# liuzhenboo/Stereo-Visual-Odometry

Hardware: AMD Instinct MI355X
Metric: stereo frames/sec on KITTI-00 1241x376; LK-kernel achieved HBM GB/s vs peak (higher is better)
Workload: dtype u8; 1 GPU; S0 synthetic KITTI-like stereo sequence 1241x376 (config #2 stand-in), FAST+LK track_mode LK_stereof2f_pnp, batched frame pairs (256 per step, 4 distinct chunks cycled), frames resident in HBM for `value`; `m1` (--full) = host-resident frames, H2D included; pairs_ok_last_step=256, parallelism=1 GPU

## Files before the change

### stereo-visual-odometry_amd/csrc/lk.hip

```cpp
#include <cstring>
#include "lk_common.h"

namespace svo {

struct ExactTile {
    static constexpr int kColDw = 29, kTileDw = 28 * kColDw;
    static constexpr int kQPairs = 23, kJPairs = 27, kJMargin = 3;
    static constexpr bool kAlignedI = true;
};
constexpr int kLdsDwPerWave = kSlots * ExactTile::kTileDw;

#ifdef SVO_LK_STAMP
__device__ unsigned long long g_lk_stamp[2 * 1024];
__device__ __forceinline__ uint32_t lk_now() { return (uint32_t)__builtin_amdgcn_readfirstlane((int)(uint32_t)__builtin_amdgcn_s_memtime()); }
#define LK_STAMP_DECL uint32_t lk_t_ = 0, lk_acc_ = 0, lk_n_ = 0
#define LK_AT(i) do { if ((i) == SVO_LK_STAMP) lk_t_ = lk_now(); else if ((i) == SVO_LK_STAMP + 1) { lk_acc_ += lk_now() - lk_t_; lk_n_++; } } while (0)
#define LK_CALL_BEGIN do { if (SVO_LK_STAMP == 8) lk_t_ = lk_now(); } while (0)
#define LK_CALL_END(lane) do { if (SVO_LK_STAMP == 8) { lk_acc_ += lk_now() - lk_t_; lk_n_++; } \
    if ((lane) == 0) { atomicAdd(&g_lk_stamp[2 * (blockIdx.x & 1023)], (unsigned long long)lk_acc_); atomicAdd(&g_lk_stamp[2 * (blockIdx.x & 1023) + 1], (unsigned long long)lk_n_); } } while (0)
#else
#define LK_STAMP_DECL
#define LK_AT(i)
#define LK_CALL_BEGIN
#define LK_CALL_END(lane)
#endif


struct PixLane { int row, seg; uint32_t onmask, qoff; };

template <bool EDGE>
__device__ __forceinline__ void patch_slot(uint32_t tile_addr, const PixLane &pl, uint32_t Wau,
                                           uint32_t Wbu, int ipx, int ipy, int w, int h,
                                           uint32_t (&IxP)[4], uint32_t (&IyP)[4], int &nIIx, int &nIIy,
                                           int &pA11, int &pA12, int &pA22)
{
    uint32_t IvP[4];
    const uint32_t Wa = Wau & pl.onmask, Wb = Wbu & pl.onmask;
    uint32_t Q12[10], DX[8], DY[8];
    scharr_columns<10, ExactTile::kColDw, EDGE>((lds_cu32 *)(size_t)(tile_addr + pl.qoff), ipx + pl.seg * 7, ipy + pl.row, w, h, Q12, DX, DY);
    int iv[8], ix[8], iy[8];
    iv[7] = ix[7] = iy[7] = 0;
    patch_samples<10>(Q12, DX, DY, Wa, Wb, iv, ix, iy);
    pA11 = 0; pA12 = 0; pA22 = 0;
    int sIIx = 0, sIIy = 0;
#pragma unroll
    for (int m = 0; m < 4; m++) {
        IvP[m] = perm_b32((uint32_t)iv[2 * m + 1], (uint32_t)iv[2 * m], 0x05040100u);
        IxP[m] = perm_b32((uint32_t)ix[2 * m + 1], (uint32_t)ix[2 * m], 0x07060302u);
        IyP[m] = perm_b32((uint32_t)iy[2 * m + 1], (uint32_t)iy[2 * m], 0x07060302u);
        pA11 = m == 0 ? dot2_0(IxP[m], IxP[m]) : dot2(IxP[m], IxP[m], pA11);
        pA12 = m == 0 ? dot2_0(IxP[m], IyP[m]) : dot2(IxP[m], IyP[m], pA12);
        pA22 = m == 0 ? dot2_0(IyP[m], IyP[m]) : dot2(IyP[m], IyP[m], pA22);
        sIIx = m == 0 ? dot2_0(IvP[m], IxP[m]) : dot2(IvP[m], IxP[m], sIIx);
        sIIy = m == 0 ? dot2_0(IvP[m], IyP[m]) : dot2(IvP[m], IyP[m], sIIy);
    }
    nIIx = -sIIx; nIIy = -sIIy;
}

__device__ __forceinline__ void mismatch_slot(const uint32_t (&C)[8], uint32_t Wa, uint32_t Wb,
                                              const uint32_t (&IxP)[4], const uint32_t (&IyP)[4], int nIIx, int nIIy,
                                              int vround, int &pb1, int &pb2)
{
    int d[7];
#pragma unroll
    for (int k = 0; k < 7; k++) d[k] = dot2(C[k + 1], Wb, dot2_sv(C[k], Wa, vround));
#pragma unroll
    for (int m = 0; m < 4; m++) {
        const uint32_t vp = m < 3 ? perm_b32((uint32_t)d[2 * m + 1], (uint32_t)d[2 * m], 0x07060302u)
                                  : (uint32_t)d[6] >> 16;
        pb1 = m == 0 ? dot2_v(vp, IxP[m], nIIx) : dot2(vp, IxP[m], pb1);
        pb2 = m == 0 ? dot2_v(vp, IyP[m], nIIy) : dot2(vp, IyP[m], pb2);
    }
}


__device__ __forceinline__ void lk_call4(const PyrGeom &g, const uint8_t *slotI, const uint8_t *slotJ, float2 prevPt,
                                         float2 &outPt, int &status, bool live, uint32_t *lds, const uint32_t *lds_wg,
                                         int wave_off, int lane)
{
    typedef ExactTile T;
    LK_STAMP_DECL;
    LK_CALL_BEGIN;
    PixLane pl;
    pl.row = min(lane / 3, kWin - 1); pl.seg = lane - (lane / 3) * 3; pl.onmask = lane < 63 ? ~0u : 0u;
    pl.qoff = (uint32_t)((pl.seg * 7 * T::kColDw + pl.row) * 4);
    asm volatile("" : "+v"(pl.onmask));

    uint32_t IxP[kSlots][4], IyP[kSlots][4];
    int nIIx[kSlots], nIIy[kSlots];
    const int lane_off = (pl.seg * 7 * T::kColDw + pl.row) * 4 + wave_off;
    const StageLane q = stage_lane<T::kColDw>(lane);
    const uint32_t lds_base = (uint32_t)(size_t)(lds_cu32 *)lds;
    const int vround = j_sample_rounding();
    status = 1;
    float nx = 0.f, ny = 0.f;
    uint32_t rI[kSlots][3][2];
    request_I<T>(rI, g, g.nlevels - 1, slotI, prevPt, live, q, lane);
    for (int level = g.nlevels - 1; level >= 0; --level) {
        LK_AT(0);
        LkLevel lv = level_begin<T>(g, level, prevPt, live, nx, ny, status);
        bool lvl_on = lv.on;
        const int w = lv.w, h = lv.h, pitch = g.pitch[level];
        const int offI = (lv.ipx - 1) - i_tile_x0<T>(lv.ipx);
        const unsigned long long m_on = __ballot(lvl_on), m_j = __ballot(lv.tx0 != kNoJTile);
        uint32_t q_src[3];
        stage_src(q_src, q, pitch);
        uint32_t rJ[kSlots][3][2];
        int pA[kSlots][3];
#pragma unroll
        for (int s = 0; s < kSlots; s++) {
            if (!((m_on >> (16 * s)) & 1ull)) continue;
            tile_store_i<T>(lds + s * T::kTileDw, rI[s], q, lane);
        }
#pragma unroll
        for (int s = 0; s < kSlots; s++) {
            if (!((m_j >> (16 * s)) & 1ull)) continue;
            tile_request<T::kJPairs>(rJ[s], g, level, pitch, slotJ, lv.tx0, lv.ty0, s, q_src, lane);
        }
        wave_lds_fence();
        LK_AT(1);
#pragma unroll
        for (int s = 0; s < kSlots; s++) {
            pA[s][0] = pA[s][1] = pA[s][2] = 0;
            if (!((m_on >> (16 * s)) & 1ull)) continue;
            const uint32_t qaddr = lds_base + (uint32_t)((s * T::kTileDw + __builtin_amdgcn_readlane(offI, 16 * s) * T::kColDw) * 4);
            const uint32_t W01s = __builtin_amdgcn_readlane(lv.WIa, 16 * s), W23s = __builtin_amdgcn_readlane(lv.WIb, 16 * s);
            const int ipxs = __builtin_amdgcn_readlane(lv.ipx, 16 * s), ipys = __builtin_amdgcn_readlane(lv.ipy, 16 * s);
            if (__builtin_expect(ipxs < 0 || ipxs + kWin >= w || ipys < 0 || ipys + kWin >= h, 0))
                patch_slot<true>(qaddr, pl, W01s, W23s, ipxs, ipys, w, h, IxP[s], IyP[s], nIIx[s], nIIy[s],
                                 pA[s][0], pA[s][1], pA[s][2]);
            else
                patch_slot<false>(qaddr, pl, W01s, W23s, ipxs, ipys, w, h, IxP[s], IyP[s], nIIx[s], nIIy[s],
                                  pA[s][0], pA[s][1], pA[s][2]);
        }
        LK_AT(2);
        wave_lds_fence();
#pragma unroll
        for (int s = 0; s < kSlots; s++) {
            if (!((m_j >> (16 * s)) & 1ull)) continue;
            tile_store_j<T, false>(lds + s * T::kTileDw, rJ[s], q, lane);
        }
        wave_lds_fence();
        float A11, A12, A22;
        {
            int v1[8], v2[8];
#pragma unroll
            for (int s = 0; s < kSlots; s++) {
                v1[2 * s] = pA[s][0]; v1[2 * s + 1] = pA[s][1];
                v2[2 * s] = pA[s][2]; v2[2 * s + 1] = 0;
            }
            const int r1 = reduce_scatter8_rows(v1, lane), r2 = reduce_scatter8_rows(v2, lane);
            A11 = wide_to_f32(quad_bcast<2>(r1), quad_bcast<0>(r1)) * kFltScale;
            A12 = wide_to_f32(quad_bcast<3>(r1), quad_bcast<1>(r1)) * kFltScale;
            A22 = wide_to_f32(quad_bcast<2>(r2), quad_bcast<0>(r2)) * kFltScale;
        }
        float Dinv;
        lvl_on = level_solve_setup(A11, A12, A22, level, lvl_on, status, Dinv);

        if (level > 0) request_I<T>(rI, g, level - 1, slotI, prevPt, live, q, lane);
        LK_AT(3);
        float pdx = 0.f, pdy = 0.f;
        bool it_on = lvl_on;
        for (int j = 0; j < kLkMaxIter; j++) {
            if (!__any(it_on)) break;
            LK_AT(4);
            const LkIter it = iter_begin<T>(lv.qx, lv.qy, w, h, level, lane, it_on, status, lv.tx0, lv.ty0);
            it_on = it.on;
            const unsigned long long m_it = __ballot(it_on), m_rs = __ballot(it.restage);
            if (__builtin_expect(m_rs != 0, 0)) {
#pragma unroll
                for (int s = 0; s < kSlots; s++) {
                    if (!((m_rs >> (16 * s)) & 1ull)) continue;
                    uint32_t r[3][2];
                    tile_request<T::kJPairs>(r, g, level, pitch, slotJ, lv.tx0, lv.ty0, s, q_src, lane);
                    tile_store_j<T, false>(lds + s * T::kTileDw, r, q, lane);
                }
                wave_lds_fence();
            }
            LK_AT(5);
            int pb[kSlots][2];
#pragma unroll
            for (int s = 0; s < kSlots; s++) {
                pb[s][0] = pb[s][1] = 0;
                if (!((m_it >> (16 * s)) & 1ull)) continue;
                const int joffs = __builtin_amdgcn_readlane(it.joff, 16 * s);
                const uint32_t Was = __builtin_amdgcn_readlane(it.Wa, 16 * s), Wbs = __builtin_amdgcn_readlane(it.Wb, 16 * s);
                lds_cu32 *pj = (lds_cu32 *)(size_t)((uint32_t)(size_t)(lds_cu32 *)lds_wg + (uint32_t)(joffs + lane_off));
                uint32_t C[8];
#pragma unroll
                for (int k = 0; k < 8; k++) C[k] = pj[k * T::kColDw];
                mismatch_slot(C, Was, Wbs, IxP[s], IyP[s], nIIx[s], nIIy[s], vround, pb[s][0], pb[s][1]);
            }
            LK_AT(6);
            float b1f, b2f;
            {
                int v[8];
#pragma unroll
                for (int s = 0; s < kSlots; s++) { v[2 * s] = pb[s][0]; v[2 * s + 1] = pb[s][1]; }
                const int r = reduce_scatter8_rows(v, lane);
                b1f = wide_to_f32(quad_bcast<2>(r), quad_bcast<0>(r)) * kFltScale;
                b2f = wide_to_f32(quad_bcast<3>(r), quad_bcast<1>(r)) * kFltScale;
            }
            it_on = iter_update(A11, A12, A22, Dinv, b1f, b2f, j, it_on, lv.qx, lv.qy, nx, ny, pdx, pdy);
            LK_AT(7);
        }
        final_window_check(nx, ny, w, h, level, live, status);
    }
    outPt = make_float2(nx, ny);
    LK_CALL_END(lane);
}

#ifndef SVO_LK_WAVES_PER_WG
#define SVO_LK_WAVES_PER_WG 1
#endif
constexpr int kLkWavesPerWg = SVO_LK_WAVES_PER_WG;
static_assert(kLkWavesPerWg == 4 || kLkWavesPerWg == 2 || kLkWavesPerWg == 1, "lk_kernel: 4, 2 or 1 waves per workgroup");
constexpr int kLkSpreadWavesPerWg = 4;

template <int W>
__global__ __launch_bounds__(64 * W) __attribute__((amdgpu_waves_per_eu(3, 3))) void lk_kernel(LkArgs a)
{
    __shared__ uint32_t lds[W * kLdsDwPerWave];
    const int wave = W == 1 ? 0 : (int)(threadIdx.x >> 6), lane = threadIdx.x & 63;
    uint32_t *my = lds + wave * kLdsDwPerWave;
    lk_track_item<W>(a, wave, lane, [&](const uint8_t *sI, const uint8_t *sJ, float2 cur, float2 &nxt, int &st, bool live) {
        lk_call4(a.g, sI, sJ, cur, nxt, st, live, my, lds, wave * (kLdsDwPerWave * 4), lane);
    });
}

__global__ __launch_bounds__(1024) void compact_kernel(CompactArgs a)
{
    __shared__ int wave_tot[16];
    __shared__ int base_s;
    const int b = blockIdx.x;
    int n = a.n_pts ? a.n_pts[b] : a.n_fixed;
    n = min(n, a.cap);
    const int lane = threadIdx.x & 63, wv = threadIdx.x >> 6;
    const int64_t o = (int64_t)b * a.pts_stride;
    if (threadIdx.x == 0) base_s = 0;
    __syncthreads();
    for (int start = 0; start < n; start += 1024) {
        int i = start + threadIdx.x;
        bool k = i < n && a.keep[o + i] != 0;
        unsigned long long m = __ballot(k);
        int rank = __popcll(m & ((1ull << lane) - 1ull));
        if (lane == 0) wave_tot[wv] = __popcll(m);
        __syncthreads();
        int pre = 0, tot = 0;
        for (int q = 0; q < 16; q++) { int t = wave_tot[q]; if (q < wv) pre += t; tot += t; }
        int dst = base_s + pre + rank;
        if (k) {
#pragma unroll
            for (int c = 0; c < 4; c++) a.out[c][o + dst] = a.in[c][o + i];
        }
        __syncthreads();
        if (threadIdx.x == 0) base_s += tot;
        __syncthreads();
    }
    if (threadIdx.x == 0) a.m_out[b] = base_s;
}

#ifdef SVO_LK_STAMP
extern "C" int svo_debug_lk_stamps(unsigned long long out[2], int reset)
{
    static unsigned long long h[2 * 1024];
    if (hipMemcpyFromSymbol(h, HIP_SYMBOL(g_lk_stamp), sizeof(h)) != hipSuccess) return -1;
    out[0] = out[1] = 0;
    for (int i = 0; i < 1024; i++) { out[0] += h[2 * i]; out[1] += h[2 * i + 1]; }
    if (reset) { memset(h, 0, sizeof(h)); if (hipMemcpyToSymbol(HIP_SYMBOL(g_lk_stamp), h, sizeof(h)) != hipSuccess) return -1; }
    return 0;
}
#endif

void launch_lk(const LkArgs &a0, int batch, int max_pts, hipStream_t st)
{
    if (max_pts <= 0 || batch <= 0) return;
    if (a0.accum != 0) { launch_lk_sse2(a0, batch, max_pts, st); return; }
    constexpr int W = kLkWavesPerWg;
// ... 24 lines not shown
```

### stereo-visual-odometry_amd/csrc/lk_common.h

```cpp
#pragma once
#include "svo_device.h"
#include "svo_kernels.h"

namespace svo {

constexpr int kSlots = 4;
constexpr int W_BITS = 14;
constexpr float kHalfWin = 10.f;
constexpr float kFltScale = 1.f / (1 << 20);
constexpr int kNoJTile = -(1 << 20);


typedef short s16x2 __attribute__((ext_vector_type(2)));
typedef unsigned short u16x2 __attribute__((ext_vector_type(2)));
typedef uint32_t u32_unaligned __attribute__((aligned(1)));
typedef const uint32_t __attribute__((address_space(3))) lds_cu32;

__device__ __forceinline__ int cv_floor(float v)
{
    int r;
    asm("v_cvt_flr_i32_f32 %0, %1" : "=v"(r) : "v"(v));
    return r;
}
__device__ __forceinline__ uint32_t perm_b32(uint32_t s0, uint32_t s1, uint32_t sel) { return __builtin_amdgcn_perm(s0, s1, sel); }
__device__ __forceinline__ int dot2(uint32_t a, uint32_t b, int c)
{
    return __builtin_amdgcn_sdot2(__builtin_bit_cast(s16x2, a), __builtin_bit_cast(s16x2, b), c, false);
}
__device__ __forceinline__ int dot2_k(uint32_t a, uint32_t b, int k)
{
    int r;
    asm("v_dot2_i32_i16 %0, %1, %2, %3" : "=v"(r) : "v"(a), "v"(b), "s"(k));
    return r;
}
__device__ __forceinline__ int dot2_0(uint32_t a, uint32_t b)
{
    int r;
    asm("v_dot2_i32_i16 %0, %1, %2, 0" : "=v"(r) : "v"(a), "v"(b));
    return r;
}
__device__ __forceinline__ uint32_t as_u32(u16x2 v) { return __builtin_bit_cast(uint32_t, v); }
__device__ __forceinline__ u16x2 as_u16x2(uint32_t v) { return __builtin_bit_cast(u16x2, v); }

__device__ __forceinline__ float wide_to_f32(int hi, int lo)
{
    return __builtin_fmaf((float)hi, 65536.f, (float)lo);
}
struct PackedWeights { uint32_t Wa, Wb; };
__device__ __forceinline__ PackedWeights bilinear_weights(float a, float b)
{
    const float magic = 12582912.f;
    const float a1 = 1.f - a, b1 = (1.f - b) * (float)(1 << W_BITS), b0 = b * (float)(1 << W_BITS);
    const uint32_t u00 = __float_as_uint(a1 * b1 + magic), u01 = __float_as_uint(a * b1 + magic),
                   u10 = __float_as_uint(a1 * b0 + magic);
    const uint32_t w11 = (uint32_t)(1 << W_BITS) + 3u * 0x4B400000u - u00 - u01 - u10;
    PackedWeights w;
    w.Wa = perm_b32(u10, u00, 0x05040100u);
    w.Wb = perm_b32(w11, u01, 0x05040100u);
    return w;
}

__device__ __forceinline__ bool window_oob(int ix, int iy, int w, int h)
{
    return (unsigned)(ix + kWin) >= (unsigned)(w + kWin) || (unsigned)(iy + kWin) >= (unsigned)(h + kWin);
}

__device__ __forceinline__ int dot2_v(uint32_t a, uint32_t b, int c)
{
    int r;
    asm("v_dot2_i32_i16 %0, %1, %2, %3" : "=v"(r) : "v"(a), "v"(b), "v"(c));
    return r;
}
__device__ __forceinline__ int dot2_sv(uint32_t a, uint32_t b_uniform, int c)
{
    int r;
    asm("v_dot2_i32_i16 %0, %1, %2, %3" : "=v"(r) : "v"(a), "s"(b_uniform), "v"(c));
    return r;
}
__device__ __forceinline__ int j_sample_rounding()
{
    int vround = 1 << (W_BITS - 5 - 1 + 7);
    asm volatile("" : "+v"(vround));
    return vround;
}

struct StageLane { int pr[3], dc4[3], dst[3]; };
template <int CS>
__device__ __forceinline__ StageLane stage_lane(int lane)
{
    StageLane q;
#pragma unroll
    for (int t = 0; t < 3; t++) {
        const int i = lane + 64 * t;
        q.pr[t] = i / 7; q.dc4[t] = 4 * (i - q.pr[t] * 7); q.dst[t] = q.dc4[t] * CS + q.pr[t];
    }
    return q;
}
__device__ __forceinline__ void stage_src(uint32_t (&src)[3], const StageLane &q, int pitch)
{
#pragma unroll
    for (int t = 0; t < 3; t++) src[t] = (uint32_t)(q.pr[t] * pitch + q.dc4[t]);
}
__device__ __forceinline__ void tile_loads(uint32_t (&r)[3][2], const uint8_t *rowA, const uint8_t *rowB, uint32_t s_off,
                                           const uint32_t (&q_src)[3], int lane, int n_items)
{
#pragma unroll
    for (int t = 0; t < 3; t++) {
        if (lane + 64 * t < n_items) {
            const uint32_t o = s_off + q_src[t];
            r[t][0] = *(const u32_unaligned *)(rowA + o); r[t][1] = *(const u32_unaligned *)(rowB + o);
        }
    }
}
template <int PAIRS>
__device__ __forceinline__ void tile_request(uint32_t (&r)[3][2], const PyrGeom &g, int level, int pitch, const uint8_t *slot,
                                             int x, int y, int s, const uint32_t (&q_src)[3], int lane)
{
// ... 28 lines not shown
                d[c * T::kColDw] = as_u32(as_u16x2(perm_b32(bot, top, 0x040c000cu + 0x01000100u * c)) >> one);
            }
        }
    }
}

template <int NC, int CS, bool EDGE>
__device__ __forceinline__ void scharr_columns(lds_cu32 *q0, int gx0, int gyA, int w, int h, uint32_t (&Q12)[NC],
                                               uint32_t (&DX)[NC - 2], uint32_t (&DY)[NC - 2])
{
    uint32_t Q01[NC], Q23[NC];
#pragma unroll
    for (int j = 0; j < NC; j++) { Q01[j] = q0[j * CS]; Q12[j] = q0[j * CS + 1]; Q23[j] = q0[j * CS + 2]; }
    uint32_t T0[NC], T1[NC];
    const u16x2 k12 = {12, 12}, k40 = {40, 40};
#pragma unroll
    for (int j = 0; j < NC; j++) {
        T0[j] = as_u32((as_u16x2(Q01[j]) + as_u16x2(Q23[j])) * k12 + as_u16x2(Q12[j]) * k40);
        T1[j] = as_u32(as_u16x2(Q23[j]) - as_u16x2(Q01[j]));
    }
#pragma unroll
    for (int c = 0; c < NC - 2; c++) {
        DX[c] = as_u32(as_u16x2(T0[c + 2]) - as_u16x2(T0[c]));
        DY[c] = as_u32((as_u16x2(T1[c]) + as_u16x2(T1[c + 2])) * k12 + as_u16x2(T1[c + 1]) * k40);
    }
    if (EDGE) {
        const int gyB = gyA + 1;
        const uint32_t rows = ((gyA >= 0 && gyA < h) ? 0x0000FFFFu : 0u) | ((gyB >= 0 && gyB < h) ? 0xFFFF0000u : 0u);
#pragma unroll
        for (int c = 0; c < NC - 2; c++) {
            const int gx = gx0 + c;
            const uint32_t mk = (gx >= 0 && gx < w) ? rows : 0u;
            DX[c] &= mk; DY[c] &= mk;
        }
    }
}
template <int NC>
__device__ __forceinline__ void patch_samples(const uint32_t (&Q12)[NC], const uint32_t (&DX)[NC - 2], const uint32_t (&DY)[NC - 2],
                                              uint32_t Wa, uint32_t Wb, int (&iv)[8], int (&ix)[8], int (&iy)[8])
{
#pragma unroll
    for (int k = 0; k < NC - 3; k++) {
        iv[k] = dot2(Q12[k + 2], Wb, dot2_k(Q12[k + 1], Wa, 1 << (W_BITS - 5 - 1))) >> (W_BITS - 5);
        ix[k] = dot2(DX[k + 1], Wb, dot2_k(DX[k], Wa, 1 << (W_BITS + 1)));
        iy[k] = dot2(DY[k + 1], Wb, dot2_k(DY[k], Wa, 1 << (W_BITS + 1)));
    }
}


template <class T> __device__ __forceinline__ int i_tile_x0(int ipx) { return T::kAlignedI ? (ipx - 1) & ~3 : ipx - 1; }

template <class T>
__device__ __forceinline__ void request_I(uint32_t (&rI)[kSlots][3][2], const PyrGeom &g, int level, const uint8_t *slotI,
                                          float2 prevPt, bool live, const StageLane &q, int lane)
{
    const float lscale = 1.f / (float)(1 << level);
    const int ipx = cv_floor(prevPt.x * lscale - kHalfWin), ipy = cv_floor(prevPt.y * lscale - kHalfWin);
    const int pitch = g.pitch[level];
    const unsigned long long m = __ballot(live && !window_oob(ipx, ipy, g.w[level], g.h[level]));
    const int x0 = i_tile_x0<T>(ipx), y0 = ipy - 1;
    uint32_t src[3];
    stage_src(src, q, pitch);
#pragma unroll
    for (int s = 0; s < kSlots; s++) {
        if (!((m >> (16 * s)) & 1ull)) continue;
        tile_request<T::kQPairs>(rI[s], g, level, pitch, slotI, x0, y0, s, src, lane);
    }
}

struct LkLevel {
    int w, h;
    int ipx, ipy;
    uint32_t WIa, WIb;
    bool on;
    float qx, qy;
    int tx0, ty0;
};
template <class T>
__device__ __forceinline__ LkLevel level_begin(const PyrGeom &g, int level, float2 prevPt, bool live, float &nx, float &ny,
                                               int &status)
{
    LkLevel v;
    v.w = g.w[level]; v.h = g.h[level];
    const float lscale = 1.f / (float)(1 << level);
    float px = prevPt.x * lscale, py = prevPt.y * lscale;
    if (level == g.nlevels - 1) { nx = px; ny = py; }
    else { nx = nx * 2.f; ny = ny * 2.f; }
    px -= kHalfWin; py -= kHalfWin;
    v.ipx = cv_floor(px); v.ipy = cv_floor(py);
    const bool oob = window_oob(v.ipx, v.ipy, v.w, v.h);
    if (live && oob && level == 0) status = 0;
    v.on = live && !oob;
    const PackedWeights wt = bilinear_weights(px - (float)v.ipx, py - (float)v.ipy);
    v.WIa = wt.Wa; v.WIb = wt.Wb;
    v.qx = nx - kHalfWin; v.qy = ny - kHalfWin;
    v.tx0 = kNoJTile; v.ty0 = 0;
    const int inx = cv_floor(v.qx), iny = cv_floor(v.qy);
    if (v.on && !window_oob(inx, iny, v.w, v.h)) { v.tx0 = inx - T::kJMargin; v.ty0 = iny - T::kJMargin; }
    return v;
}

__device__ __forceinline__ bool level_solve_setup(float A11, float A12, float A22, int level, bool lvl_on, int &status, float &Dinv)
{
    const float D = A11 * A22 - A12 * A12;
    const float minEig = (A22 + A11 - sqrtf((A11 - A22) * (A11 - A22) + 4.f * A12 * A12)) /
                         (float)(2 * kWin * kWin);
    const bool degenerate = minEig < 0.001f || D < 1.1920929e-07f;
    if (lvl_on && degenerate && level == 0) status = 0;
    Dinv = 1.f / D;
    return lvl_on && !degenerate;
}

struct LkIter {
    bool on;
    uint32_t Wa, Wb;
    int joff;
    bool restage;
};
template <class T>
__device__ __forceinline__ LkIter iter_begin(float qx, float qy, int w, int h, int level, int lane, bool it_on, int &status,
                                             int &tx0, int &ty0)
{
    LkIter it;
    const int inx = cv_floor(qx), iny = cv_floor(qy);
    if (it_on && window_oob(inx, iny, w, h)) {
        if (level == 0) status = 0;
        it_on = false;
    }
    const PackedWeights wj = bilinear_weights(qx - (float)inx, qy - (float)iny);
    it.Wa = wj.Wa; it.Wb = wj.Wb;
    int cx = inx - tx0, cy = iny - ty0;
    it.restage = it_on && ((unsigned)cx > (unsigned)(2 * T::kJMargin) || (unsigned)cy > (unsigned)(2 * T::kJMargin));
    if (it.restage) { tx0 = inx - T::kJMargin; ty0 = iny - T::kJMargin; cx = T::kJMargin; cy = T::kJMargin; }
    it.joff = ((int)__umul24((unsigned)cx, T::kColDw) + cy + (lane >> 4) * T::kTileDw) * 4;
    it.on = it_on;
    return it;
}

__device__ __forceinline__ bool iter_update(float A11, float A12, float A22, float Dinv, float b1f, float b2f, int j, bool it_on,
                                            float &qx, float &qy, float &nx, float &ny, float &pdx, float &pdy)
{
    const float dlx = (A12 * b2f - A22 * b1f) * Dinv;
    const float dly = (A12 * b1f - A11 * b2f) * Dinv;
    const float dd = dlx * dlx + dly * dly;
    bool conv = dd <= 0.9999e-4f;
    if (__builtin_expect(__any(it_on && !conv && dd < 1.0001e-4f), 0)) {
        asm volatile("" ::: "memory");
        conv = (double)dlx * (double)dlx + (double)dly * (double)dly <= 0.01 * 0.01;
    }
    if (it_on) {
        qx += dlx; qy += dly;
        nx = qx + kHalfWin; ny = qy + kHalfWin;
        if (conv) it_on = false;
        else if (j > 0 && fabsf(dlx + pdx) <= 0.01f && fabsf(dly + pdy) <= 0.01f) {
            nx -= dlx * 0.5f; ny -= dly * 0.5f;
            it_on = false;
        }
        pdx = dlx; pdy = dly;
    }
    return it_on;
}

__device__ __forceinline__ void final_window_check(float nx, float ny, int w, int h, int level, bool live, int &status)
{
    if (live && status && level == 0) {
        const int fx = cv_floor(nx - kHalfWin), fy = cv_floor(ny - kHalfWin);
        if (window_oob(fx, fy, w, h)) status = 0;
    }
}

struct LkItem { int b, bx; };
__device__ __forceinline__ LkItem lk_item_of_workgroup(const LkArgs &a)
{
    const int n_aware = (a.batch & ~7) * a.gx;
    LkItem it;
    if ((int)blockIdx.x < n_aware) {
        const int xcd = blockIdx.x & 7, slot_id = blockIdx.x >> 3;
        it.b = (slot_id / a.gx) * 8 + xcd; it.bx = slot_id % a.gx;
    } else {
        const int r = blockIdx.x - n_aware;
        it.b = (a.batch & ~7) + r / a.gx; it.bx = r % a.gx;
    }
    return it;
}

template <int W, class Call>
__device__ __forceinline__ void lk_track_item(const LkArgs &a, int wave, int lane, Call &&lk_call)
{
    const LkItem item = lk_item_of_workgroup(a);
    const int b = item.b, slot = lane >> 4;
    int n = a.n_pts ? a.n_pts[b] : a.n_fixed;
    n = min(n, a.cap);
    int spw = kSlots;
    if (a.spread) spw = min(kSlots, max(1, (n + a.gx * W - 1) / (a.gx * W)));
    for (int first = (item.bx * W + wave) * spw; first < n; first += a.gx * W * spw) {
        const int idx = first + slot;
        const bool valid = slot < spw && idx < n;
        const bool writer = valid && lane == 16 * slot;
        const int64_t po = (int64_t)b * a.pts_stride + (valid ? idx : first);
        const float2 p0 = a.pts_in[po];
        float2 cur = p0, nxt;
        bool outside = p0.x < 0 || p0.y < 0, bad = false, noepi = false;
        bool live = valid;
        float prev_y = p0.y;
#pragma nounroll
        for (int c = 0; c < a.ncalls; c++) {
            const uint8_t *sI = a.prev[c] + (int64_t)b * a.slot_stride;
            const uint8_t *sJ = a.next[c] + (int64_t)b * a.slot_stride;
            int st;
            lk_call(sI, sJ, cur, nxt, st, live);
            if (writer && live) {
                a.pts_out[c][po] = nxt;
                a.status[c][po] = (uint8_t)st;
            }
            if (live) {
                outside = outside || nxt.x < 0 || nxt.y < 0;
                bad = bad || st == 0;
                if (c == 0 || c == 2) noepi = noepi || (double)fabsf(prev_y - nxt.y) > a.match_err;
                prev_y = nxt.y;
                cur = nxt;
            }
            if (a.ncalls == 4 && (outside || bad || noepi)) live = false;
            if (!__any(live)) break;
        }
        if (a.ncalls == 4 && writer) a.keep[po] = !(outside || bad || noepi);
        wave_lds_fence();
    }
}

}
```

### stereo-visual-odometry_amd/csrc/lk_sse2.hip

```cpp
#include "lk_common.h"

namespace svo {

constexpr int kCS2 = 26, kJMargin2 = 2;
constexpr int kQPairs2 = 23, kJPairs2 = kWin + 2 * kJMargin2;
constexpr int kTileDw2 = 26 * kCS2, kTileSpill = 2 * kCS2;
constexpr int kTilesDw = kSlots * kTileDw2;
struct ChainTile {
    static constexpr int kColDw = kCS2, kTileDw = kTileDw2;
    static constexpr int kQPairs = kQPairs2, kJPairs = kJPairs2, kJMargin = kJMargin2;
    static constexpr bool kAlignedI = false;
};
constexpr int kStageDw = 576;
constexpr int kTailY = 0, kTailX = 416;
__device__ constexpr int kChainOff[8] = {108, 196, 372, 284, 328, 240, 524, 152};
constexpr int kAq0 = kTileSpill;
__host__ __device__ constexpr int a_stride(bool simd128) { return simd128 ? 84 : 108; }
__host__ __device__ constexpr int a_tail_base(bool simd128) { return kAq0 + 4 * a_stride(simd128); }
constexpr int kLdsDwSse2 = kTilesDw + kSlots * kStageDw + 16;
constexpr int kDumpB = kChainOff[0] + 43, kDumpA = kStageDw - 1;
constexpr int kStageDwL = 960, kTailYL = 180, kTailXL = 468;
__device__ constexpr int kChainOffL[8] = {88, 584, 0, 764, 676, 288, 376, 860};
constexpr int kLdsDwLegacy = kTilesDw + kSlots * kStageDwL + 16;
constexpr int kDumpBL = kChainOffL[0] + 87, kDumpAL = kStageDwL - 1;
// ... 196 lines not shown
#pragma unroll
    for (int i = 0; i < 3; i++)
#pragma unroll
        for (int e = 0; e < 4; e++)
            if (4 * i + e >= first && 4 * i + e < last) {
                const f32x2 f = {(float)(short)(q[i][e] & 0xFFFFu), (float)((int)q[i][e] >> 16)};
                d = pk_fma(f, f, d);
                m = __builtin_fmaf(f.x, f.y, m);
            }
}
__device__ __forceinline__ void chain_a(const Sse2Lane &L, float &s11, float &s12, float &s22)
{
    lds_cu32x4 *p = (lds_cu32x4 *)(size_t)L.ca;
    f32x2 d = {0.f, 0.f}, d21, d84 = {0.f, 0.f};
    float m = 0.f, m21, m84 = 0.f;
    u32x4 q[3], n[3];
#pragma unroll
    for (int i = 0; i < 3; i++) q[i] = p[i];
#pragma unroll
    for (int i = 0; i < 3; i++) n[i] = p[3 + i];
    asm volatile("" ::: "memory");
    a_terms(d, m, q, 0, 12);
#pragma unroll
    for (int i = 0; i < 3; i++) q[i] = p[6 + i];
    asm volatile("" ::: "memory");
    a_terms(d, m, n, 0, 9);
    d21 = d; m21 = m;
    a_terms(d, m, n, 9, 12);
#pragma nounroll
    for (int turn = 0; turn < 3; turn++, p += 6) {
#pragma unroll
        for (int i = 0; i < 3; i++) n[i] = p[9 + i];
        asm volatile("" ::: "memory");
        a_terms(d, m, q, 0, 12);
        if (turn == 2) { d84 = d; m84 = m; }
#pragma unroll
        for (int i = 0; i < 3; i++) q[i] = p[12 + i];
        asm volatile("" ::: "memory");
        a_terms(d, m, n, 0, 12);
    }
    a_terms(d, m, q, 0, 9);
    s11 = L.a_sel == 0 ? d21.x : (L.a_sel == 1 ? d84.x : d.x);
    s12 = L.a_sel == 0 ? m21 : (L.a_sel == 1 ? m84 : m);
    s22 = L.a_sel == 0 ? d21.y : (L.a_sel == 1 ? d84.y : d.y);
}
__device__ __forceinline__ float combine_a(float r)
{
    const float u = ((r + row_shl<1>(r)) + row_shl<2>(r)) + row_shl<3>(r);
    return row_first(row_shl<4>(r) + u);
}

template <bool LEGACY>
__device__ __forceinline__ void lk_call4_sse2(const PyrGeom &g, const uint8_t *slotI, const uint8_t *slotJ, float2 prevPt,
                                              float2 &outPt, int &status, bool live, uint32_t *lds, int lane,
                                              const Sse2Lane &L)
{
    typedef ChainTile T;
    uint32_t IvP[kSlots][4], IxP[kSlots][4], IyP[kSlots][4], Ix4[kSlots], Iy4[kSlots];
    const StageLane q = stage_lane<T::kColDw>(lane);
    const uint32_t lds_base = (uint32_t)(size_t)(lds_cu32 *)lds;
    const int vround = j_sample_rounding();
    status = 1;
    float nx = 0.f, ny = 0.f;
    uint32_t rI[kSlots][3][2];
    request_I<T>(rI, g, g.nlevels - 1, slotI, prevPt, live, q, lane);
    for (int level = g.nlevels - 1; level >= 0; --level) {
        LkLevel lv = level_begin<T>(g, level, prevPt, live, nx, ny, status);
        bool lvl_on = lv.on;
        const int w = lv.w, h = lv.h, pitch = g.pitch[level];
        const unsigned long long m_on = __ballot(lvl_on), m_j = __ballot(lv.tx0 != kNoJTile);
        uint32_t q_src[3];
        stage_src(q_src, q, pitch);
        uint32_t rJ[kSlots][3][2];
#pragma unroll
        for (int s = 0; s < kSlots; s++) {
            if (!((m_on >> (16 * s)) & 1ull)) continue;
            tile_store_i<T>(lds + s * T::kTileDw, rI[s], q, lane);
        }
#pragma unroll
        for (int s = 0; s < kSlots; s++) {
            if (!((m_j >> (16 * s)) & 1ull)) continue;
            tile_request<T::kJPairs>(rJ[s], g, level, pitch, slotJ, lv.tx0, lv.ty0, s, q_src, lane);
        }
        wave_lds_fence();
#pragma unroll
        for (int s = 0; s < kSlots; s++) {
            if (!((m_on >> (16 * s)) & 1ull)) continue;
            const uint32_t qaddr = lds_base + (uint32_t)(s * T::kTileDw * 4);
            const uint32_t W01s = __builtin_amdgcn_readlane(lv.WIa, 16 * s), W23s = __builtin_amdgcn_readlane(lv.WIb, 16 * s);
            const int ipxs = __builtin_amdgcn_readlane(lv.ipx, 16 * s), ipys = __builtin_amdgcn_readlane(lv.ipy, 16 * s);
            uint32_t Aw[8];
            if (__builtin_expect(ipxs < 0 || ipxs + kWin >= w || ipys < 0 || ipys + kWin >= h, 0))
                patch_slot8<true>(qaddr, L, W01s, W23s, ipxs, ipys, w, h, IvP[s], IxP[s], IyP[s], Ix4[s], Iy4[s], Aw);
            else
                patch_slot8<false>(qaddr, L, W01s, W23s, ipxs, ipys, w, h, IvP[s], IxP[s], IyP[s], Ix4[s], Iy4[s], Aw);
            const uint32_t so = (uint32_t)(s * stage_dw<LEGACY>() * 4);
#pragma unroll
            for (int i = 0; i < 8; i++) lds_store(L.wa[i] + so, Aw[i]);
        }
        wave_lds_fence();
#pragma unroll
        for (int s = 0; s < kSlots; s++) {
            if (!((m_j >> (16 * s)) & 1ull)) continue;
            tile_store_j<T, false>(lds + s * T::kTileDw, rJ[s], q, lane);
        }
        float A11, A12, A22;
        {
            float r11, r12, r22;
            chain_a(L, r11, r12, r22);
            A11 = combine_a(r11) * kFltScale;
            A12 = combine_a(r12) * kFltScale;
            A22 = combine_a(r22) * kFltScale;
        }
        wave_lds_fence();
        float Dinv;
        lvl_on = level_solve_setup(A11, A12, A22, level, lvl_on, status, Dinv);

        if (level > 0) request_I<T>(rI, g, level - 1, slotI, prevPt, live, q, lane);
        float pdx = 0.f, pdy = 0.f;
        bool it_on = lvl_on;
        for (int j = 0; j < kLkMaxIter; j++) {
            if (!__any(it_on)) break;
            const LkIter it = iter_begin<T>(lv.qx, lv.qy, w, h, level, lane, it_on, status, lv.tx0, lv.ty0);
            it_on = it.on;
            const unsigned long long m_it = __ballot(it_on), m_rs = __ballot(it.restage);
            if (__builtin_expect(m_rs != 0, 0)) {
#pragma unroll
                for (int s = 0; s < kSlots; s++) {
                    if (!((m_rs >> (16 * s)) & 1ull)) continue;
                    uint32_t r[3][2];
                    tile_request<T::kJPairs>(r, g, level, pitch, slotJ, lv.tx0, lv.ty0, s, q_src, lane);
                    tile_store_j<T, true>(lds + s * T::kTileDw, r, q, lane);
                }
                wave_lds_fence();
            }
#pragma unroll
            for (int s = 0; s < kSlots; s++) {
                if (!((m_it >> (16 * s)) & 1ull)) continue;
                const int joffs = __builtin_amdgcn_readlane(it.joff, 16 * s);
                const uint32_t Was = __builtin_amdgcn_readlane(it.Wa, 16 * s), Wbs = __builtin_amdgcn_readlane(it.Wb, 16 * s);
                lds_cu32 *pj = (lds_cu32 *)(size_t)(lds_base + (uint32_t)joffs + L.qoff);
                uint32_t C[9];
#pragma unroll
                for (int k = 0; k < 9; k++) C[k] = pj[k * T::kColDw];
                float v[16];
                mismatch_slot8<LEGACY>(C, Was, Wbs, IvP[s], IxP[s], IyP[s], Ix4[s], Iy4[s], vround, v);
                const uint32_t so = (uint32_t)(s * stage_dw<LEGACY>() * 4);
#pragma unroll
                for (int t = 0; t < (LEGACY ? 16 : 10); t++) lds_store(L.wb[t] + so, __float_as_uint(v[t]));
            }
            wave_lds_fence();
            float b1f, b2f;
            {
                const float r = chain_b<LEGACY>(L);
                const float bb = r + row_shl<1>(r);
                const float u = bb + row_shl<2>(bb);
                const float f = r + row_shl<1>(u);
                b1f = row_first(f) * kFltScale;
                b2f = row_first(row_shl<8>(f)) * kFltScale;
            }
            wave_lds_fence();
            it_on = iter_update(A11, A12, A22, Dinv, b1f, b2f, j, it_on, lv.qx, lv.qy, nx, ny, pdx, pdy);
        }
        final_window_check(nx, ny, w, h, level, live, status);
    }
    outPt = make_float2(nx, ny);
}

template <bool LEGACY>
__global__ __launch_bounds__(64) __attribute__((amdgpu_waves_per_eu(2, 2))) void lk_sse2_kernel(LkArgs a)
{
    __shared__ __attribute__((aligned(16))) uint32_t lds[LEGACY ? kLdsDwLegacy : kLdsDwSse2];
    const int lane = threadIdx.x & 63;
    const Sse2Lane L = make_lane<LEGACY>(lane, (uint32_t)(size_t)(lds_cu32 *)lds, a.accum == 2);
    lk_track_item<1>(a, 0, lane, [&](const uint8_t *sI, const uint8_t *sJ, float2 cur, float2 &nxt, int &st, bool live) {
        lk_call4_sse2<LEGACY>(a.g, sI, sJ, cur, nxt, st, live, lds, lane, L);
    });
}

void launch_lk_sse2(const LkArgs &a0, int batch, int max_pts, hipStream_t st)
{
    if (max_pts <= 0 || batch <= 0) return;
    const int waves = (max_pts + kSlots - 1) / kSlots;
    LkArgs a = a0;
    a.gx = waves < 768 ? waves : 768;
    a.spread = 0;
    if (batch < 4) {
        const int room = 2048 / batch;
        a.gx = max_pts < room ? max_pts : room;
        a.spread = 1;
    }
    a.batch = batch;
    if (a.accum == 3) {
        if (batch < 4) {
            const int room = 1536 / batch;
            a.gx = max_pts < room ? max_pts : room;
        }
        hipLaunchKernelGGL(lk_sse2_kernel<true>, dim3(batch * a.gx), dim3(64), 0, st, a);
    } else {
        hipLaunchKernelGGL(lk_sse2_kernel<false>, dim3(batch * a.gx), dim3(64), 0, st, a);
    }
}

}
```

Before: 18650 stereo pairs/s.

## Represent LK per-lane predicates as wave-wide lane masks instead of bools

```diff
diff --git a/stereo-visual-odometry_amd/csrc/lk.hip b/stereo-visual-odometry_amd/csrc/lk.hip
--- a/stereo-visual-odometry_amd/csrc/lk.hip
+++ b/stereo-visual-odometry_amd/csrc/lk.hip
@@ -74,8 +74,11 @@
 }
 
 
+__device__ __forceinline__ void undefined_sums(int &x, int &y) { asm("" : "=v"(x), "=v"(y)); }
+__device__ __forceinline__ void undefined_sums(int &x, int &y, int &z) { asm("" : "=v"(x), "=v"(y), "=v"(z)); }
+
 __device__ __forceinline__ void lk_call4(const PyrGeom &g, const uint8_t *slotI, const uint8_t *slotJ, float2 prevPt,
-                                         float2 &outPt, int &status, bool live, uint32_t *lds, const uint32_t *lds_wg,
+                                         float2 &outPt, lanemask &status, lanemask live, uint32_t *lds, const uint32_t *lds_wg,
                                          int wave_off, int lane)
 {
     typedef ExactTile T;
@@ -92,37 +95,37 @@
     const StageLane q = stage_lane<T::kColDw>(lane);
     const uint32_t lds_base = (uint32_t)(size_t)(lds_cu32 *)lds;
     const int vround = j_sample_rounding();
-    status = 1;
+    status = ~0ull;
     float nx = 0.f, ny = 0.f;
     uint32_t rI[kSlots][3][2];
     request_I<T>(rI, g, g.nlevels - 1, slotI, prevPt, live, q, lane);
     for (int level = g.nlevels - 1; level >= 0; --level) {
         LK_AT(0);
         LkLevel lv = level_begin<T>(g, level, prevPt, live, nx, ny, status);
-        bool lvl_on = lv.on;
+        lanemask lvl_on = lv.on;
         const int w = lv.w, h = lv.h, pitch = g.pitch[level];
         const int offI = (lv.ipx - 1) - i_tile_x0<T>(lv.ipx);
-        const unsigned long long m_on = __ballot(lvl_on), m_j = __ballot(lv.tx0 != kNoJTile);
+        const lanemask m_on = lvl_on, m_j = lv.j_staged;
         uint32_t q_src[3];
         stage_src(q_src, q, pitch);
         uint32_t rJ[kSlots][3][2];
         int pA[kSlots][3];
 #pragma unroll
         for (int s = 0; s < kSlots; s++) {
-            if (!((m_on >> (16 * s)) & 1ull)) continue;
+            if (!slot_bit(m_on, s)) continue;
             tile_store_i<T>(lds + s * T::kTileDw, rI[s], q, lane);
         }
 #pragma unroll
         for (int s = 0; s < kSlots; s++) {
-            if (!((m_j >> (16 * s)) & 1ull)) continue;
+            if (!slot_bit(m_j, s)) continue;
             tile_request<T::kJPairs>(rJ[s], g, level, pitch, slotJ, lv.tx0, lv.ty0, s, q_src, lane);
         }
         wave_lds_fence();
         LK_AT(1);
 #pragma unroll
         for (int s = 0; s < kSlots; s++) {
-            pA[s][0] = pA[s][1] = pA[s][2] = 0;
-            if (!((m_on >> (16 * s)) & 1ull)) continue;
+            undefined_sums(pA[s][0], pA[s][1], pA[s][2]);
+            if (!slot_bit(m_on, s)) continue;
             const uint32_t qaddr = lds_base + (uint32_t)((s * T::kTileDw + __builtin_amdgcn_readlane(offI, 16 * s) * T::kColDw) * 4);
             const uint32_t W01s = __builtin_amdgcn_readlane(lv.WIa, 16 * s), W23s = __builtin_amdgcn_readlane(lv.WIb, 16 * s);
             const int ipxs = __builtin_amdgcn_readlane(lv.ipx, 16 * s), ipys = __builtin_amdgcn_readlane(lv.ipy, 16 * s);
@@ -137,7 +140,7 @@
         wave_lds_fence();
 #pragma unroll
         for (int s = 0; s < kSlots; s++) {
-            if (!((m_j >> (16 * s)) & 1ull)) continue;
+            if (!slot_bit(m_j, s)) continue;
             tile_store_j<T, false>(lds + s * T::kTileDw, rJ[s], q, lane);
         }
         wave_lds_fence();
@@ -160,17 +163,17 @@
         if (level > 0) request_I<T>(rI, g, level - 1, slotI, prevPt, live, q, lane);
         LK_AT(3);
         float pdx = 0.f, pdy = 0.f;
-        bool it_on = lvl_on;
+        lanemask it_on = lvl_on;
         for (int j = 0; j < kLkMaxIter; j++) {
-            if (!__any(it_on)) break;
+            if (!it_on) break;
             LK_AT(4);
             const LkIter it = iter_begin<T>(lv.qx, lv.qy, w, h, level, lane, it_on, status, lv.tx0, lv.ty0);
             it_on = it.on;
-            const unsigned long long m_it = __ballot(it_on), m_rs = __ballot(it.restage);
+            const lanemask m_it = it_on, m_rs = it.restage;
             if (__builtin_expect(m_rs != 0, 0)) {
 #pragma unroll
                 for (int s = 0; s < kSlots; s++) {
-                    if (!((m_rs >> (16 * s)) & 1ull)) continue;
+                    if (!slot_bit(m_rs, s)) continue;
                     uint32_t r[3][2];
                     tile_request<T::kJPairs>(r, g, level, pitch, slotJ, lv.tx0, lv.ty0, s, q_src, lane);
                     tile_store_j<T, false>(lds + s * T::kTileDw, r, q, lane);
@@ -181,8 +184,8 @@
             int pb[kSlots][2];
 #pragma unroll
             for (int s = 0; s < kSlots; s++) {
-                pb[s][0] = pb[s][1] = 0;
-                if (!((m_it >> (16 * s)) & 1ull)) continue;
+                undefined_sums(pb[s][0], pb[s][1]);
+                if (!slot_bit(m_it, s)) continue;
                 const int joffs = __builtin_amdgcn_readlane(it.joff, 16 * s);
                 const uint32_t Was = __builtin_amdgcn_readlane(it.Wa, 16 * s), Wbs = __builtin_amdgcn_readlane(it.Wb, 16 * s);
                 lds_cu32 *pj = (lds_cu32 *)(size_t)((uint32_t)(size_t)(lds_cu32 *)lds_wg + (uint32_t)(joffs + lane_off));
@@ -223,7 +226,7 @@
     __shared__ uint32_t lds[W * kLdsDwPerWave];
     const int wave = W == 1 ? 0 : (int)(threadIdx.x >> 6), lane = threadIdx.x & 63;
     uint32_t *my = lds + wave * kLdsDwPerWave;
-    lk_track_item<W>(a, wave, lane, [&](const uint8_t *sI, const uint8_t *sJ, float2 cur, float2 &nxt, int &st, bool live) {
+    lk_track_item<W>(a, wave, lane, [&](const uint8_t *sI, const uint8_t *sJ, float2 cur, float2 &nxt, lanemask &st, lanemask live) {
         lk_call4(a.g, sI, sJ, cur, nxt, st, live, my, lds, wave * (kLdsDwPerWave * 4), lane);
     });
 }
diff --git a/stereo-visual-odometry_amd/csrc/lk_common.h b/stereo-visual-odometry_amd/csrc/lk_common.h
--- a/stereo-visual-odometry_amd/csrc/lk_common.h
+++ b/stereo-visual-odometry_amd/csrc/lk_common.h
@@ -60,9 +60,23 @@
     return w;
 }
 
-__device__ __forceinline__ bool window_oob(int ix, int iy, int w, int h)
-{
-    return (unsigned)(ix + kWin) >= (unsigned)(w + kWin) || (unsigned)(iy + kWin) >= (unsigned)(h + kWin);
+typedef unsigned long long lanemask;
+enum { kIcmpUgt = 34, kIcmpUge = 35 };
+enum { kFcmpOgt = 2, kFcmpOlt = 4, kFcmpOle = 5 };
+__device__ __forceinline__ lanemask mask_ugt(unsigned a, unsigned b) { return __builtin_amdgcn_uicmp(a, b, kIcmpUgt); }
+__device__ __forceinline__ lanemask mask_uge(unsigned a, unsigned b) { return __builtin_amdgcn_uicmp(a, b, kIcmpUge); }
+__device__ __forceinline__ lanemask mask_lt(float a, float b) { return __builtin_amdgcn_fcmpf(a, b, kFcmpOlt); }
+__device__ __forceinline__ lanemask mask_le(float a, float b) { return __builtin_amdgcn_fcmpf(a, b, kFcmpOle); }
+__device__ __forceinline__ lanemask mask_le(double a, double b) { return __builtin_amdgcn_fcmp(a, b, kFcmpOle); }
+__device__ __forceinline__ lanemask mask_gt(double a, double b) { return __builtin_amdgcn_fcmp(a, b, kFcmpOgt); }
+__device__ __forceinline__ bool lane_of(lanemask m) { return __builtin_amdgcn_inverse_ballot_w64(m); }
+__device__ __forceinline__ int select(int a, int b, lanemask m) { return lane_of(m) ? a : b; }
+__device__ __forceinline__ float select(float a, float b, lanemask m) { return lane_of(m) ? a : b; }
+__device__ __forceinline__ bool slot_bit(lanemask m, int s) { return (m >> (16 * s)) & 1ull; }
+
+__device__ __forceinline__ lanemask window_oob(int ix, int iy, int w, int h)
+{
+    return mask_uge((unsigned)(ix + kWin), (unsigned)(w + kWin)) | mask_uge((unsigned)(iy + kWin), (unsigned)(h + kWin));
 }
 
 __device__ __forceinline__ int dot2_v(uint32_t a, uint32_t b, int c)
@@ -197,18 +211,18 @@
 
 template <class T>
 __device__ __forceinline__ void request_I(uint32_t (&rI)[kSlots][3][2], const PyrGeom &g, int level, const uint8_t *slotI,
-                                          float2 prevPt, bool live, const StageLane &q, int lane)
+                                          float2 prevPt, lanemask live, const StageLane &q, int lane)
 {
     const float lscale = 1.f / (float)(1 << level);
     const int ipx = cv_floor(prevPt.x * lscale - kHalfWin), ipy = cv_floor(prevPt.y * lscale - kHalfWin);
     const int pitch = g.pitch[level];
-    const unsigned long long m = __ballot(live && !window_oob(ipx, ipy, g.w[level], g.h[level]));
+    const lanemask m = live & ~window_oob(ipx, ipy, g.w[level], g.h[level]);
     const int x0 = i_tile_x0<T>(ipx), y0 = ipy - 1;
     uint32_t src[3];
     stage_src(src, q, pitch);
 #pragma unroll
     for (int s = 0; s < kSlots; s++) {
-        if (!((m >> (16 * s)) & 1ull)) continue;
+        if (!slot_bit(m, s)) continue;
         tile_request<T::kQPairs>(rI[s], g, level, pitch, slotI, x0, y0, s, src, lane);
     }
 }
@@ -217,13 +231,14 @@
     int w, h;
     int ipx, ipy;
     uint32_t WIa, WIb;
-    bool on;
+    lanemask on;
     float qx, qy;
     int tx0, ty0;
+    lanemask j_staged;
 };
 template <class T>
-__device__ __forceinline__ LkLevel level_begin(const PyrGeom &g, int level, float2 prevPt, bool live, float &nx, float &ny,
-                                               int &status)
+__device__ __forceinline__ LkLevel level_begin(const PyrGeom &g, int level, float2 prevPt, lanemask live, float &nx, float &ny,
+                                               lanemask &status)
 {
     LkLevel v;
     v.w = g.w[level]; v.h = g.h[level];
@@ -233,84 +248,81 @@
     else { nx = nx * 2.f; ny = ny * 2.f; }
     px -= kHalfWin; py -= kHalfWin;
     v.ipx = cv_floor(px); v.ipy = cv_floor(py);
-    const bool oob = window_oob(v.ipx, v.ipy, v.w, v.h);
-    if (live && oob && level == 0) status = 0;
-    v.on = live && !oob;
+    const lanemask oob = window_oob(v.ipx, v.ipy, v.w, v.h);
+    if (level == 0) status &= ~(live & oob);
+    v.on = live & ~oob;
     const PackedWeights wt = bilinear_weights(px - (float)v.ipx, py - (float)v.ipy);
     v.WIa = wt.Wa; v.WIb = wt.Wb;
     v.qx = nx - kHalfWin; v.qy = ny - kHalfWin;
-    v.tx0 = kNoJTile; v.ty0 = 0;
     const int inx = cv_floor(v.qx), iny = cv_floor(v.qy);
-    if (v.on && !window_oob(inx, iny, v.w, v.h)) { v.tx0 = inx - T::kJMargin; v.ty0 = iny - T::kJMargin; }
+    v.j_staged = v.on & ~window_oob(inx, iny, v.w, v.h);
+    v.tx0 = select(inx - T::kJMargin, kNoJTile, v.j_staged); v.ty0 = select(iny - T::kJMargin, 0, v.j_staged);
     return v;
 }
 
-__device__ __forceinline__ bool level_solve_setup(float A11, float A12, float A22, int level, bool lvl_on, int &status, float &Dinv)
+__device__ __forceinline__ lanemask level_solve_setup(float A11, float A12, float A22, int level, lanemask lvl_on, lanemask &status,
+                                                      float &Dinv)
 {
     const float D = A11 * A22 - A12 * A12;
     const float minEig = (A22 + A11 - sqrtf((A11 - A22) * (A11 - A22) + 4.f * A12 * A12)) /
                          (float)(2 * kWin * kWin);
-    const bool degenerate = minEig < 0.001f || D < 1.1920929e-07f;
-    if (lvl_on && degenerate && level == 0) status = 0;
+    const lanemask degenerate = mask_lt(minEig, 0.001f) | mask_lt(D, 1.1920929e-07f);
+    if (level == 0) status &= ~(lvl_on & degenerate);
     Dinv = 1.f / D;
-    return lvl_on && !degenerate;
+    return lvl_on & ~degenerate;
 }
 
 struct LkIter {
-    bool on;
+    lanemask on;
     uint32_t Wa, Wb;
     int joff;
-    bool restage;
+    lanemask restage;
 };
 template <class T>
-__device__ __forceinline__ LkIter iter_begin(float qx, float qy, int w, int h, int level, int lane, bool it_on, int &status,
+__device__ __forceinline__ LkIter iter_begin(float qx, float qy, int w, int h, int level, int lane, lanemask it_on, lanemask &status,
                                              int &tx0, int &ty0)
 {
     LkIter it;
     const int inx = cv_floor(qx), iny = cv_floor(qy);
-    if (it_on && window_oob(inx, iny, w, h)) {
-        if (level == 0) status = 0;
-        it_on = false;
-    }
+    const lanemask oob = window_oob(inx, iny, w, h);
+    if (level == 0) status &= ~(it_on & oob);
+    it_on &= ~oob;
     const PackedWeights wj = bilinear_weights(qx - (float)inx, qy - (float)iny);
     it.Wa = wj.Wa; it.Wb = wj.Wb;
-    int cx = inx - tx0, cy = iny - ty0;
-    it.restage = it_on && ((unsigned)cx > (unsigned)(2 * T::kJMargin) || (unsigned)cy > (unsigned)(2 * T::kJMargin));
-    if (it.restage) { tx0 = inx - T::kJMargin; ty0 = iny - T::kJMargin; cx = T::kJMargin; cy = T::kJMargin; }
+    it.restage = it_on & (mask_ugt((unsigned)(inx - tx0), (unsigned)(2 * T::kJMargin)) |
+                          mask_ugt((unsigned)(iny - ty0), (unsigned)(2 * T::kJMargin)));
+    tx0 = select(inx - T::kJMargin, tx0, it.restage); ty0 = select(iny - T::kJMargin, ty0, it.restage);
+    const int cx = inx - tx0, cy = iny - ty0;
     it.joff = ((int)__umul24((unsigned)cx, T::kColDw) + cy + (lane >> 4) * T::kTileDw) * 4;
     it.on = it_on;
     return it;
 }
 
-__device__ __forceinline__ bool iter_update(float A11, float A12, float A22, float Dinv, float b1f, float b2f, int j, bool it_on,
-                                            float &qx, float &qy, float &nx, float &ny, float &pdx, float &pdy)
+__device__ __forceinline__ lanemask iter_update(float A11, float A12, float A22, float Dinv, float b1f, float b2f, int j, lanemask it_on,
+                                                float &qx, float &qy, float &nx, float &ny, float &pdx, float &pdy)
 {
     const float dlx = (A12 * b2f - A22 * b1f) * Dinv;
     const float dly = (A12 * b1f - A11 * b2f) * Dinv;
     const float dd = dlx * dlx + dly * dly;
-    bool conv = dd <= 0.9999e-4f;
-    if (__builtin_expect(__any(it_on && !conv && dd < 1.0001e-4f), 0)) {
+    lanemask conv = mask_le(dd, 0.9999e-4f);
+    if (__builtin_expect((it_on & ~conv & mask_lt(dd, 1.0001e-4f)) != 0, 0)) {
         asm volatile("" ::: "memory");
-        conv = (double)dlx * (double)dlx + (double)dly * (double)dly <= 0.01 * 0.01;
-    }
-    if (it_on) {
-        qx += dlx; qy += dly;
-        nx = qx + kHalfWin; ny = qy + kHalfWin;
-        if (conv) it_on = false;
-        else if (j > 0 && fabsf(dlx + pdx) <= 0.01f && fabsf(dly + pdy) <= 0.01f) {
-            nx -= dlx * 0.5f; ny -= dly * 0.5f;
-            it_on = false;
-        }
-        pdx = dlx; pdy = dly;
-    }
-    return it_on;
-}
-
-__device__ __forceinline__ void final_window_check(float nx, float ny, int w, int h, int level, bool live, int &status)
-{
-    if (live && status && level == 0) {
+        conv = mask_le((double)dlx * (double)dlx + (double)dly * (double)dly, 0.01 * 0.01);
+    }
+    qx += dlx; qy += dly;
+    const lanemask osc = j > 0 ? it_on & ~conv & mask_le(fabsf(dlx + pdx), 0.01f) & mask_le(fabsf(dly + pdy), 0.01f) : 0ull;
+    const float sx = qx + kHalfWin, sy = qy + kHalfWin;
+    nx = select(select(sx - dlx * 0.5f, sx, osc), nx, it_on);
+    ny = select(select(sy - dly * 0.5f, sy, osc), ny, it_on);
+    pdx = dlx; pdy = dly;
+    return it_on & ~conv & ~osc;
+}
+
+__device__ __forceinline__ void final_window_check(float nx, float ny, int w, int h, int level, lanemask live, lanemask &status)
+{
+    if (level == 0) {
         const int fx = cv_floor(nx - kHalfWin), fy = cv_floor(ny - kHalfWin);
-        if (window_oob(fx, fy, w, h)) status = 0;
+        status &= ~(live & window_oob(fx, fy, w, h));
     }
 }
 
@@ -345,30 +357,28 @@
         const int64_t po = (int64_t)b * a.pts_stride + (valid ? idx : first);
         const float2 p0 = a.pts_in[po];
         float2 cur = p0, nxt;
-        bool outside = p0.x < 0 || p0.y < 0, bad = false, noepi = false;
-        bool live = valid;
+        lanemask outside = mask_lt(p0.x, 0.f) | mask_lt(p0.y, 0.f), bad = 0, noepi = 0;
+        lanemask live = __ballot(valid);
         float prev_y = p0.y;
 #pragma nounroll
         for (int c = 0; c < a.ncalls; c++) {
             const uint8_t *sI = a.prev[c] + (int64_t)b * a.slot_stride;
             const uint8_t *sJ = a.next[c] + (int64_t)b * a.slot_stride;
-            int st;
+            lanemask st;
             lk_call(sI, sJ, cur, nxt, st, live);
-            if (writer && live) {
+            if (writer && lane_of(live)) {
                 a.pts_out[c][po] = nxt;
-                a.status[c][po] = (uint8_t)st;
+                a.status[c][po] = (uint8_t)select(1, 0, st);
             }
-            if (live) {
-                outside = outside || nxt.x < 0 || nxt.y < 0;
-                bad = bad || st == 0;
-                if (c == 0 || c == 2) noepi = noepi || (double)fabsf(prev_y - nxt.y) > a.match_err;
-                prev_y = nxt.y;
-                cur = nxt;
-            }
-            if (a.ncalls == 4 && (outside || bad || noepi)) live = false;
-            if (!__any(live)) break;
-        }
-        if (a.ncalls == 4 && writer) a.keep[po] = !(outside || bad || noepi);
+            outside |= live & (mask_lt(nxt.x, 0.f) | mask_lt(nxt.y, 0.f));
+            bad |= live & ~st;
+            if (c == 0 || c == 2) noepi |= live & mask_gt((double)fabsf(prev_y - nxt.y), a.match_err);
+            prev_y = select(nxt.y, prev_y, live);
+            cur.x = select(nxt.x, cur.x, live); cur.y = select(nxt.y, cur.y, live);
+            if (a.ncalls == 4) live &= ~(outside | bad | noepi);
+            if (!live) break;
+        }
+        if (a.ncalls == 4 && writer) a.keep[po] = !lane_of(outside | bad | noepi);
         wave_lds_fence();
     }
 }
diff --git a/stereo-visual-odometry_amd/csrc/lk_sse2.hip b/stereo-visual-odometry_amd/csrc/lk_sse2.hip
--- a/stereo-visual-odometry_amd/csrc/lk_sse2.hip
+++ b/stereo-visual-odometry_amd/csrc/lk_sse2.hip
@@ -272,7 +272,7 @@
 
 template <bool LEGACY>
 __device__ __forceinline__ void lk_call4_sse2(const PyrGeom &g, const uint8_t *slotI, const uint8_t *slotJ, float2 prevPt,
-                                              float2 &outPt, int &status, bool live, uint32_t *lds, int lane,
+                                              float2 &outPt, lanemask &status, lanemask live, uint32_t *lds, int lane,
                                               const Sse2Lane &L)
 {
     typedef ChainTile T;
@@ -280,32 +280,32 @@
     const StageLane q = stage_lane<T::kColDw>(lane);
     const uint32_t lds_base = (uint32_t)(size_t)(lds_cu32 *)lds;
     const int vround = j_sample_rounding();
-    status = 1;
+    status = ~0ull;
     float nx = 0.f, ny = 0.f;
     uint32_t rI[kSlots][3][2];
     request_I<T>(rI, g, g.nlevels - 1, slotI, prevPt, live, q, lane);
     for (int level = g.nlevels - 1; level >= 0; --level) {
         LkLevel lv = level_begin<T>(g, level, prevPt, live, nx, ny, status);
-        bool lvl_on = lv.on;
+        lanemask lvl_on = lv.on;
         const int w = lv.w, h = lv.h, pitch = g.pitch[level];
-        const unsigned long long m_on = __ballot(lvl_on), m_j = __ballot(lv.tx0 != kNoJTile);
+        const lanemask m_on = lvl_on, m_j = lv.j_staged;
         uint32_t q_src[3];
         stage_src(q_src, q, pitch);
         uint32_t rJ[kSlots][3][2];
 #pragma unroll
         for (int s = 0; s < kSlots; s++) {
-            if (!((m_on >> (16 * s)) & 1ull)) continue;
+            if (!slot_bit(m_on, s)) continue;
             tile_store_i<T>(lds + s * T::kTileDw, rI[s], q, lane);
         }
 #pragma unroll
         for (int s = 0; s < kSlots; s++) {
-            if (!((m_j >> (16 * s)) & 1ull)) continue;
+            if (!slot_bit(m_j, s)) continue;
             tile_request<T::kJPairs>(rJ[s], g, level, pitch, slotJ, lv.tx0, lv.ty0, s, q_src, lane);
         }
         wave_lds_fence();
 #pragma unroll
         for (int s = 0; s < kSlots; s++) {
-            if (!((m_on >> (16 * s)) & 1ull)) continue;
+            if (!slot_bit(m_on, s)) continue;
             const uint32_t qaddr = lds_base + (uint32_t)(s * T::kTileDw * 4);
             const uint32_t W01s = __builtin_amdgcn_readlane(lv.WIa, 16 * s), W23s = __builtin_amdgcn_readlane(lv.WIb, 16 * s);
             const int ipxs = __builtin_amdgcn_readlane(lv.ipx, 16 * s), ipys = __builtin_amdgcn_readlane(lv.ipy, 16 * s);
@@ -321,7 +321,7 @@
         wave_lds_fence();
 #pragma unroll
         for (int s = 0; s < kSlots; s++) {
-            if (!((m_j >> (16 * s)) & 1ull)) continue;
+            if (!slot_bit(m_j, s)) continue;
             tile_store_j<T, false>(lds + s * T::kTileDw, rJ[s], q, lane);
         }
         float A11, A12, A22;
@@ -338,16 +338,16 @@
 
         if (level > 0) request_I<T>(rI, g, level - 1, slotI, prevPt, live, q, lane);
         float pdx = 0.f, pdy = 0.f;
-        bool it_on = lvl_on;
+        lanemask it_on = lvl_on;
         for (int j = 0; j < kLkMaxIter; j++) {
-            if (!__any(it_on)) break;
+            if (!it_on) break;
             const LkIter it = iter_begin<T>(lv.qx, lv.qy, w, h, level, lane, it_on, status, lv.tx0, lv.ty0);
             it_on = it.on;
-            const unsigned long long m_it = __ballot(it_on), m_rs = __ballot(it.restage);
+            const lanemask m_it = it_on, m_rs = it.restage;
             if (__builtin_expect(m_rs != 0, 0)) {
 #pragma unroll
                 for (int s = 0; s < kSlots; s++) {
-                    if (!((m_rs >> (16 * s)) & 1ull)) continue;
+                    if (!slot_bit(m_rs, s)) continue;
                     uint32_t r[3][2];
                     tile_request<T::kJPairs>(r, g, level, pitch, slotJ, lv.tx0, lv.ty0, s, q_src, lane);
                     tile_store_j<T, true>(lds + s * T::kTileDw, r, q, lane);
@@ -356,7 +356,7 @@
             }
 #pragma unroll
             for (int s = 0; s < kSlots; s++) {
-                if (!((m_it >> (16 * s)) & 1ull)) continue;
+                if (!slot_bit(m_it, s)) continue;
                 const int joffs = __builtin_amdgcn_readlane(it.joff, 16 * s);
                 const uint32_t Was = __builtin_amdgcn_readlane(it.Wa, 16 * s), Wbs = __builtin_amdgcn_readlane(it.Wb, 16 * s);
                 lds_cu32 *pj = (lds_cu32 *)(size_t)(lds_base + (uint32_t)joffs + L.qoff);
@@ -393,7 +393,7 @@
     __shared__ __attribute__((aligned(16))) uint32_t lds[LEGACY ? kLdsDwLegacy : kLdsDwSse2];
     const int lane = threadIdx.x & 63;
     const Sse2Lane L = make_lane<LEGACY>(lane, (uint32_t)(size_t)(lds_cu32 *)lds, a.accum == 2);
-    lk_track_item<1>(a, 0, lane, [&](const uint8_t *sI, const uint8_t *sJ, float2 cur, float2 &nxt, int &st, bool live) {
+    lk_track_item<1>(a, 0, lane, [&](const uint8_t *sI, const uint8_t *sJ, float2 cur, float2 &nxt, lanemask &st, lanemask live) {
         lk_call4_sse2<LEGACY>(a.g, sI, sJ, cur, nxt, st, live, lds, lane, L);
     });
 }
```

Result: faster. 19300 stereo pairs/s (median of 6 runs) (+3.5%).
